# microsoft/VidTok

Hardware: AMD Instinct MI355X
Metric: encode+decode frames/sec, vidtok_kl_causal_488_4chn 17x256x256 (higher is better)
Workload: dtype bf16; 1 GPU; vidtok_kl_causal_488_4chn forward (encode+KL+decode), bf16, B=4 clips/GPU, 17x256x256; global_batch=4, launch=hipGraph replay (engine graph cache)

## Files before the change

### include/vidtok_amd.h

```cpp
#ifndef VIDTOK_AMD_H
#define VIDTOK_AMD_H

#include <stddef.h>
#include <stdint.h>

#ifdef __cplusplus
extern "C" {
#endif

typedef void* vt_stream;

typedef enum vt_status {
  VT_OK = 0,
  VT_ERR_ARG = -1,
  VT_ERR_HIP = -2,
  VT_ERR_UNSUPPORTED = -3
} vt_status;

typedef enum vt_dtype { VT_F32 = 0, VT_BF16 = 1, VT_I32 = 2, VT_BF16X3 = 3 , VT_F16 = 4 } vt_dtype;

typedef enum vt_tmode {
  VT_TPAD_ZERO = 0,
  VT_TPAD_REPLICATE = 1,
  VT_TPAD_CACHE = 2,
// ... 36 lines not shown
  int32_t ldy;
  int32_t KT, KH, KW;
  int32_t st, sh, sw;
  int32_t pt, ph, pw;
  int32_t tmode, ncache;
  int32_t ups_t, ups_s;
  int32_t res_mode;
  int32_t res_tshift;
  int32_t Tr, ldr;
  int32_t out_layout;
  int32_t t_trim;
  int32_t dtype;
  int32_t out_dtype;
  int32_t nbatch;
  int32_t ln_mode;
  int32_t ln_keep_y;
  int32_t ldn;
  int32_t yt_mul, yt_off;
  int32_t ys_mul, ys_oh, ys_ow;
  float ln_eps;
  int64_t xs_z, ws_z, ys_z, rs_z;
  void* work;
  int64_t work_bytes;
} vt_conv_desc;

int vt_conv(const vt_conv_desc* d, vt_stream stream);
int64_t vt_conv_work_bytes(const vt_conv_desc* d);
int vt_conv_plan(const vt_conv_desc* d, int32_t* out8);
int vt_conv_profile(const vt_conv_desc* d, uint64_t* stamps_out, vt_stream stream);
int vt_conv_desc_size(void);

int vt_time_upsample3_supported(const vt_conv_desc* u);
int vt_time_upsample3(const vt_conv_desc* u, const void* v, int32_t ldv, vt_stream stream);

typedef struct vt_tblock_desc {
  const void* x;
  void* y;
  void* n_out;
  const void* w1; const float* b1;
  const void* w2; const float* b2;
  const float* norm1_gamma; const float* norm1_beta;
  const float* norm2_gamma; const float* norm2_beta;
  const float* next_gamma; const float* next_beta;
  int32_t dtype;
  int32_t C, ld;
  int32_t B, T;
  int64_t HW;
  int32_t tmode;
  int32_t keep_y;
  int32_t ln_next_mode;
  float eps;
  int32_t cache_offset;
  void* cache1;
  void* cache2;
} vt_tblock_desc;

int vt_tblock_desc_size(void);
int vt_temporal_block_supported(const vt_tblock_desc* d);
int vt_temporal_block(const vt_tblock_desc* d, vt_stream stream);
int vt_temporal_block_profile(const vt_tblock_desc* d, uint64_t* stamps_out, vt_stream stream);

int vt_layernorm_act(const void* x, int in_dtype, int64_t ldx, void* y, int out_dtype, int64_t ldy,
                     const float* gamma, const float* beta, int64_t M, int32_t C, float eps,
                     int32_t silu, vt_stream stream);

typedef enum { VT_GN_FRAME = 0, VT_GN_PIXEL = 1, VT_GN_CLIP = 2 } vt_gn_scope;
// ... 214 lines not shown
```

### vidtok_amd/csrc/conv_igemm.hip

```cpp
#include <algorithm>
#include <atomic>
#include <type_traits>

#include "conv_select.h"

namespace {

template <typename H>
__global__ __launch_bounds__(256) void splitk_reduce_kernel(const float* __restrict__ part, int planes, long long M, int Cout, const float* __restrict__ bias,
                                                            const H* __restrict__ res, H* __restrict__ y) {
  const long long n8 = M * (Cout / 8);
  const long long plane = M * (long long)Cout;
  for (long long i = (long long)blockIdx.x * blockDim.x + threadIdx.x; i < n8; i += (long long)gridDim.x * blockDim.x) {
    const long long e = i * 8;
    const int c = (int)(e % Cout);
    float v[8];
    {
      const f32x4 a = *reinterpret_cast<const f32x4*>(part + e), b = *reinterpret_cast<const f32x4*>(part + e + 4);
#pragma unroll
      for (int k = 0; k < 4; ++k) { v[k] = a[k]; v[4 + k] = b[k]; }
    }
    for (int pz = 1; pz < planes; ++pz) {
      const f32x4 a = *reinterpret_cast<const f32x4*>(part + pz * plane + e), b = *reinterpret_cast<const f32x4*>(part + pz * plane + e + 4);
#pragma unroll
      for (int k = 0; k < 4; ++k) { v[k] += a[k]; v[4 + k] += b[k]; }
    }
    if (bias) {
      const f32x4 a = *reinterpret_cast<const f32x4*>(bias + c), b = *reinterpret_cast<const f32x4*>(bias + c + 4);
#pragma unroll
      for (int k = 0; k < 4; ++k) { v[k] += a[k]; v[4 + k] += b[k]; }
    }
    if (res) {
      Oct<H> r;
      r.load(res + e);
#pragma unroll
      for (int k = 0; k < 8; ++k) v[k] = r.get(k) + v[k];
    }
    Oct<H>::store(y + e, v);
  }
}

int launch_igemm(int dtype, bool out_f32, const ConvArgs& a, const IgemmVariant& v, int nbatch, void* stream) {
  switch (dtype) {
    case VT_F32: return vt_igemm_dispatch_f32(&a, &v, nbatch, stream);
    case VT_BF16X3: return vt_igemm_dispatch_x3(&a, &v, nbatch, stream);
    case VT_F16: return vt_igemm_dispatch_f16(&a, &v, nbatch, out_f32 ? 1 : 0, stream);
    default: return vt_igemm_dispatch_bf16(&a, &v, nbatch, out_f32 ? 1 : 0, stream);
  }
}

bool splitk_runs(const ConvPlan& p, const ConvArgs& a, const vt_conv_desc* d, bool sized) {
  if (p.kernel != CONV_IGEMM || p.splitk_planes == 0 || d->work == nullptr) return false;
  return !sized || (d->work_bytes >= (int64_t)p.splitk_planes * a.M * a.Cout * 4 && (reinterpret_cast<uintptr_t>(d->work) & 15) == 0);
}

int launch_splitk(const vt_conv_desc* d, const ConvArgs& a_in, const ConvPlan& p, hipStream_t stream) {
  const int planes = p.splitk_planes;
  ConvArgs a = a_in;
  a.ksplit = a.KT == 3 ? 1 : 2;
  a.plane_bytes = (unsigned)((a.KT == 3 ? a.KH * a.KW : a.KW) * a.Cin * 2);
  a.y = reinterpret_cast<char*>(d->work);
  a.bias = nullptr;
  a.res = nullptr; a.res_mode = VT_RES_NONE;
  a.ln_mode = 0;
  a.xs_z = 0; a.ws_z = 0; a.rs_z = 0;
  a.ys_z = (long long)a.M * a.ldy;
  int rc = launch_igemm(d->dtype, true, a, p.split, planes, stream);
  if (rc != VT_OK) return rc;
  const long long n8 = (long long)a.M * (a.Cout / 8);
  const unsigned grid = (unsigned)std::min<long long>((n8 + 255) / 256, 4096);
  const void* res = a_in.res_mode == VT_RES_ADD ? a_in.res : nullptr;
  if (d->dtype == VT_F16)
    hipLaunchKernelGGL(splitk_reduce_kernel<f16_t>, dim3(grid), dim3(256), 0, stream, reinterpret_cast<const float*>(d->work), planes, (long long)a.M, a.Cout, a_in.bias,
                       reinterpret_cast<const f16_t*>(res), reinterpret_cast<f16_t*>(a_in.y));
  else
    hipLaunchKernelGGL(splitk_reduce_kernel<bf16_t>, dim3(grid), dim3(256), 0, stream, reinterpret_cast<const float*>(d->work), planes, (long long)a.M, a.Cout, a_in.bias,
                       reinterpret_cast<const bf16_t*>(res), reinterpret_cast<bf16_t*>(a_in.y));
  VT_CHECK_LAUNCH();
  return VT_OK;
}

}

extern "C" int vt_conv_max_lds_bytes(void) { return 163840; }

extern "C" int vt_conv_plan(const vt_conv_desc* d, int32_t* out8) {
  VT_CHECK_ARG(out8 != nullptr, "vt_conv_plan: null output");
  ConvArgs a;
  ConvPlan p;
  const int rc = conv_decide(d, a, p);
  if (rc != VT_OK) return rc;
  out8[4] = p.ln_fused ? 1 : 0;
  out8[5] = 1;
  out8[6] = p.kernel;
  out8[7] = 0;
  switch (p.kernel) {
    case CONV_NARROW:
      vt_conv_narrow_plan(&a, out8);
      out8[5] = p.narrow_mode == 2 ? 2 : 1;
      break;
    case CONV_WS2:
      out8[0] = 64; out8[1] = 128; out8[2] = 8;
      out8[3] = (a.Wo / 16) * (a.Ho / 4) * a.B * a.To;
      break;
    case CONV_IN8:
      out8[0] = 128; out8[1] = 128; out8[2] = 4;
      out8[3] = a.M / 128;
      out8[7] = 1;
      break;
    case CONV_IGEMM: {
      const TileShape& t = kTileShapes[p.igemm.tile];
      out8[0] = t.bm(); out8[1] = t.bn(); out8[2] = t.waves();
// ... 16 lines not shown
  a.prof_mode = vt_opt(OPT_WS_PROF_MODE);
  if (p.kernel == CONV_WS2) return vt_ws2_launch(&a, d->dtype, stream_);
  VT_CHECK_ARG(p.kernel == CONV_IGEMM && ((d->dtype == VT_BF16 && d->out_dtype == VT_BF16) || d->dtype == VT_BF16X3) && d->ln_mode == 0 &&
                   p.igemm.tile == TILE_256x256,
               "vt_conv_profile: bf16 / split-bf16 launches on the 256 x 256 tile without LayerNorm, or on the weight-stationary kernel");
  return launch_igemm(d->dtype, false, a, p.igemm, p.nbatch, stream_);
}

extern "C" int64_t vt_conv_work_bytes(const vt_conv_desc* d) {
  ConvArgs a;
  ConvPlan p;
  if (conv_decide(d, a, p) != VT_OK || p.kernel != CONV_IGEMM) return 0;
  return (int64_t)p.splitk_planes * a.M * a.Cout * 4;
}

extern "C" int vt_conv(const vt_conv_desc* d, vt_stream stream_) {
  ConvArgs a;
  ConvPlan p;
  int rc = conv_decide(d, a, p);
  if (rc != VT_OK) return rc;
  switch (p.kernel) {
    case CONV_WS2: return vt_ws2_launch(&a, d->dtype, stream_);
    case CONV_NARROW: return vt_conv_narrow_launch(&a, stream_, p.narrow_mode);
    case CONV_IN8: return vt_conv_in8_launch(&a, d->dtype, stream_);
    case CONV_IGEMM: break;
  }
  rc = splitk_runs(p, a, d, true) ? launch_splitk(d, a, p, reinterpret_cast<hipStream_t>(stream_))
                                  : launch_igemm(d->dtype, d->out_dtype == VT_F32, a, p.igemm, p.nbatch, stream_);
  if (rc != VT_OK || d->ln_mode == 0 || p.ln_fused) return rc;
  return vt_layernorm_act(d->y, d->out_dtype, d->ldy, d->ln_out, d->out_dtype, d->ldn, d->ln_gamma, d->ln_beta, a.M, d->Cout,
                          d->ln_eps, d->ln_mode == 2 ? 1 : 0, stream_);
}

extern "C" int vt_time_upsample3_supported(const vt_conv_desc* u) {
  ConvArgs a;
  ConvPlan p;
  if (conv_decide(u, a, p) != VT_OK) return 0;
  return tup3_eligible(u, a, p) ? 1 : 0;
}

extern "C" int vt_time_upsample3(const vt_conv_desc* u, const void* v, int32_t ldv, vt_stream stream_) {
  ConvArgs a;
  ConvPlan p;
  const int rc = conv_decide(u, a, p);
  if (rc != VT_OK) return rc;
  VT_CHECK_ARG(tup3_eligible(u, a, p), "vt_time_upsample3: descriptor not covered (ask vt_time_upsample3_supported; the parity launches of vt_conv serve it)");
  VT_CHECK_ARG(v != nullptr && (reinterpret_cast<uintptr_t>(v) & 15) == 0 && ldv >= u->Cout && ldv % 8 == 0,
               "vt_time_upsample3: v must be 16-byte aligned with ldv = %d >= Cout and a multiple of 8", ldv);
  a.pair_v = reinterpret_cast<const char*>(v);
  a.ldv = ldv;
  const IgemmVariant pair = {TILE_256x256, true, 2, 2, kRowBytes};
  return launch_igemm(u->dtype, false, a, pair, 1, stream_);
}

extern "C" int vt_conv_act(const vt_conv_desc* d, int32_t act, vt_stream stream_) {
  VT_CHECK_ARG(act == VT_ACT_RELU, "vt_conv_act: act %d (VT_ACT_RELU = %d is the one activation)", act, VT_ACT_RELU);
  ConvArgs a;
  ConvPlan p;
  const int rc = conv_decide(d, a, p, nullptr, act);
  if (rc != VT_OK) return rc;
  VT_CHECK_ARG(d->dtype != VT_BF16X3 && d->out_dtype == d->dtype, "vt_conv_act: fp32, bf16 or fp16 arithmetic with results in the same type");
  VT_CHECK_ARG(d->out_layout == VT_NDHWC && d->res_mode == VT_RES_NONE && d->ln_mode == 0 && p.nbatch == 1 && a.yt_mul == 1 && a.ys_mul == 1,
               "vt_conv_act: NDHWC output without residual, LayerNorm, batching or interleave");
  return vt_igemm_dispatch_relu(&a, &p.igemm, d->dtype, stream_);
}
```

### vidtok_amd/csrc/model.cpp

```cpp
#include <hip/hip_runtime.h>
#include <stdint.h>
#include <string.h>

#include <algorithm>
#include <cmath>
#include <map>
#include <memory>
#include <set>
#include <string>
#include <vector>

#include "../../include/vidtok_amd.h"

void vt_set_error(const char* fmt, ...);

namespace {

struct Fail {
  int code;
};
#define M_CHECK(cond, ...)        \
  do {                            \
    if (!(cond)) {                \
      vt_set_error(__VA_ARGS__);  \
// ... 394 lines not shown
  }
  auto standins = [&](vt_conv_desc& q) {
    if (!c.dry) return;
    q.x = q.w = q.y = (void*)16;
    if (q.res_mode != VT_RES_NONE) q.res = (void*)16;
    if (q.res_mode == VT_RES_MIX) q.mix_factor = (const float*)16;
    if (q.tmode == VT_TPAD_CACHE) q.cache = (void*)16;
    if (q.ln_mode != 0) { q.ln_gamma = q.ln_beta = (const float*)16; q.ln_out = (void*)16; }
  };
  if (o.ln_optional && d.ln_mode != 0) {
    vt_conv_desc q = d;
    standins(q);
    int32_t plan[8];
    if (q.ln_out == nullptr) q.ln_out = (void*)16;
    if (!(vt_conv_plan(&q, plan) == VT_OK && plan[4] == 1)) {
      d.ln_gamma = d.ln_beta = nullptr; d.ln_out = nullptr; d.ln_mode = 0;
      r.n = Tens(); r.norm = nullptr;
    }
  }
  if (o.tup3_probe) {
    vt_conv_desc q = d;
    standins(q);
    if (q.ln_mode != 0 && q.ln_out == nullptr) q.ln_out = (void*)16;
    r.tup3 = vt_time_upsample3_supported(&q) == 1;
  }
  if (o.plan_only) return r;
  if (o.tup3_v) {
    if (!c.dry) M_CALL(vt_time_upsample3(&d, o.tup3_v->p, o.tup3_v->ld, c.stream));
    return r;
  }
  {
    vt_conv_desc q = d;
    standins(q);
    const int64_t wb = ((x.dt == VT_BF16 || x.dt == VT_F16) && (g.kt == 3 || g.kh == 3)) ? vt_conv_work_bytes(&q) : 0;
    if (wb > 0) {
      d.work = c.cur->alloc((size_t)wb, c.dry);
      d.work_bytes = wb;
    }
  }
  if (!c.dry) M_CALL(vt_conv(&d, c.stream));
  if (ln_after) {
    M_CHECK(!o.out && !o.ncthw, "vt_model: GroupNorm of an interleaved / NCTHW result");
    r.n = o.ln.norm->of(c, r.y, o.ln.silu, cout);
    r.norm = o.ln.norm; r.silu = o.ln.silu;
  }
  return r;
}

void gather(Ctx& c, const char* src, int Ts, char* dst, int Td, int t0, const std::vector<int>& idx, int B, int64_t frame_elems, int es) {
  for (size_t j0 = 0; j0 < idx.size(); j0 += 128) {
    int32_t part[128];
    const int n = (int)std::min<size_t>(128, idx.size() - j0);
    for (int j = 0; j < n; ++j) part[j] = idx[j0 + j];
    if (!c.dry)
      M_CALL(vt_gather_frames(src, dst + (size_t)(t0 + (int)j0) * frame_elems * es, es, B, frame_elems, (int64_t)Ts * frame_elems, (int64_t)Td * frame_elems, part, n, c.stream));
  }
}

void update_cache(Ctx& c, CState& st, const Tens& x, int P) {
  if (P == 0) return;
  Model* m = c.m;
  const int T = x.T, off = st.offset, es = (int)esize(x.dt);
  const int64_t fr = (int64_t)x.H * x.W * x.ld;
  std::vector<int> sx, sc;
  int jx = -1, jc = -1;
  for (int j = 0; j < P; ++j) {
    const int q = T - off + j;
    M_CHECK(q >= 0, "vt_model: chunk of %d frames is shorter than its cache offset %d", T, off);
    if (q >= P) { if (jx < 0) jx = j; sx.push_back(q - P); }
    else if (m->first_chunk) { if (jx < 0) jx = j; sx.push_back(0); }
// ... 1419 lines not shown
```

### vidtok_amd/csrc/options.cpp

```cpp
#include "options.h"

#include <stdlib.h>
#include <string.h>

#include <atomic>
#include <mutex>

#include "../../include/vidtok_amd.h"

void vt_set_error(const char* fmt, ...);

namespace {
struct OptDef {
  const char* name;
  int dflt;
};
const OptDef kDefs[OPT_COUNT] = {
    {"conv_buf", 1},        {"conv_tinner", 1},     {"conv_ldsepi", 1},      {"conv_ws", 2},
    {"conv_narrow", 1},     {"conv_tile", 0},       {"conv_tile_min", 128},  {"conv_fuse_ln", 1}, {"conv_fuse_ln256", 1},
    {"tblock_fused", 1},    {"tblock_prof_mode", 0},
    {"conv_deep", 1},       {"ws_prof_mode", 0},    {"attn_flash", 1},      {"conv_splitk", 1},
    {"conv_tskip", 1},      {"conv_in8", 1},        {"conv_tup_ln", 1},     {"conv_nt_mb", 64},
    {"conv_tup3", 1},
};
std::atomic<int> g_val[OPT_COUNT];
std::once_flag g_once;

int env_default(int id) {
  char var[64] = "VT_";
  size_t n = 3;
  for (const char* s = kDefs[id].name; *s && n + 1 < sizeof(var); ++s) var[n++] = (*s >= 'a' && *s <= 'z') ? (char)(*s - 32) : *s;
  var[n] = 0;
  const char* e = getenv(var);
  return e ? atoi(e) : kDefs[id].dflt;
}
void init_all() {
  for (int i = 0; i < OPT_COUNT; ++i) g_val[i].store(env_default(i), std::memory_order_relaxed);
}
int find(const char* name) {
  if (!name) return -1;
  for (int i = 0; i < OPT_COUNT; ++i)
    if (strcmp(name, kDefs[i].name) == 0) return i;
  return -1;
}
}

int vt_opt(int id) {
  std::call_once(g_once, init_all);
  return g_val[id].load(std::memory_order_relaxed);
}

extern "C" int vt_set_option(const char* name, int32_t value) {
  const int id = find(name);
  if (id < 0) {
    vt_set_error("vt_set_option: unknown option '%s'", name ? name : "(null)");
    return VT_ERR_ARG;
// ... 25 lines not shown
```

### vidtok_amd/csrc/options.h

```cpp
#pragma once

enum VtOpt {
  OPT_CONV_BUF = 0,
  OPT_CONV_TINNER,
  OPT_CONV_LDSEPI,
  OPT_CONV_WS,
  OPT_CONV_NARROW,
  OPT_CONV_TILE,
  OPT_CONV_TILE_MIN,
  OPT_CONV_FUSE_LN,
  OPT_CONV_FUSE_LN256,
  OPT_TBLOCK_FUSED,
  OPT_TBLOCK_PROF_MODE,
  OPT_CONV_DEEP,
  OPT_WS_PROF_MODE,
  OPT_ATTN_FLASH,
  OPT_CONV_SPLITK,
  OPT_CONV_TSKIP,
  OPT_CONV_IN8,
  OPT_CONV_TUP_LN,
  OPT_CONV_NT_MB,
  OPT_CONV_TUP3,
  OPT_COUNT
};

int vt_opt(int id);
```

### vidtok_amd/lib.py

```python
import ctypes as C
import os

import torch

_HERE = os.path.dirname(os.path.abspath(__file__))
LIB_PATH = os.path.join(_HERE, "libvidtok_amd.so")

VT_F32, VT_BF16, VT_I32, VT_BF16X3, VT_F16 = 0, 1, 2, 3, 4
VT_TPAD_ZERO, VT_TPAD_REPLICATE, VT_TPAD_CACHE, VT_TPAD_ZERO_BACK = 0, 1, 2, 3
VT_GN_FRAME, VT_GN_PIXEL, VT_GN_CLIP = 0, 1, 2
VT_RES_NONE, VT_RES_ADD, VT_RES_MIX = 0, 1, 2
VT_NDHWC, VT_NCTHW = 0, 1
VT_ACT_RELU = 1
VT_LPIPS_CLAMP_Y, VT_LPIPS_ROUNDTRIP, VT_LPIPS_UNIT = 1, 2, 4
VT_SESSION_ENCODE, VT_SESSION_DECODE = 0, 1


class VtError(RuntimeError):
    pass


class ConvDesc(C.Structure):

    _fields_ = (
# ... 91 lines not shown
    "vt_create": (C.c_int, [C.POINTER(ModelConfig), _I32, C.POINTER(_P)]),
    "vt_destroy": (C.c_int, [_P]),
    "vt_load_weight": (C.c_int, [_P, C.c_char_p, _P, C.POINTER(_I64), _I32]),
    "vt_weight_count": (C.c_int, [_P]),
    "vt_weight_name": (C.c_char_p, [_P, _I32]),
    "vt_weight_shape": (C.c_int, [_P, _I32, C.POINTER(_I64), C.POINTER(_I32)]),
    "vt_workspace_bytes": (_I64, [_P, _I32, _I32, _I32, _I32]),
    "vt_latent_dims": (C.c_int, [_P, _I32, _I32, _I32, C.POINTER(_I32)]),
    "vt_encode": (C.c_int, [_P, _P, _I32, _I32, _I32, _I32, _P, _P, _I64, _P]),
    "vt_regularize_kl": (C.c_int, [_P, _P, _P, _P, _P, _I32, _I32, _I32, _I32, _P]),
    "vt_regularize_fsq": (C.c_int, [_P, _P, _P, _P, _I32, _I32, _I32, _I32, _P]),
    "vt_indices_to_latent": (C.c_int, [_P, _P, _P, _I32, _I32, _I32, _I32, _P]),
    "vt_decode": (C.c_int, [_P, _P, _I32, _I32, _I32, _I32, _P, _P, _I64, _P]),
    "vt_reset_cache": (C.c_int, [_P]),
    "vt_prepare": (C.c_int, [_P]),
    "vt_regularize_fsq_aux": (C.c_int, [_P, _P, _I32, _I32, _I32, _I32, _F, _P, _P, _P]),
    "vt_tile_latent_frames": (_I32, [_P, _I32, _I32]),
    "vt_tile_workspace_bytes": (_I64, [_P, _I32, _I32, _I32, _I32, _I32, _I32]),
    "vt_tile_encode": (C.c_int, [_P, _P, _I32, _I32, _I32, _I32, _I32, _P, _P, _I64, _P]),
    "vt_tile_decode": (C.c_int, [_P, _P, _I32, _I32, _I32, _I32, _I32, _I32, _P, _P, _I64, _P]),
    "vt_session_create": (C.c_int, [_P, _I32, _I32, _I32, _I32, _I32, _I32, C.POINTER(_P)]),
    "vt_session_workspace_bytes": (_I64, [_P]),
    "vt_session_push": (C.c_int, [_P, _P, _I32, _P, _I32, C.POINTER(_I32), _P, _I64, _P]),
    "vt_session_finish": (C.c_int, [_P, _P, _I32, C.POINTER(_I32), _P, _I64, _P]),
    "vt_session_destroy": (C.c_int, [_P]),
    "vt_copy_segments": (C.c_int, [_P, _I32, _I64, _P]),
    "vt_conv": (C.c_int, [C.POINTER(ConvDesc), _P]),
    "vt_conv_desc_size": (C.c_int, []),
    "vt_conv_work_bytes": (_I64, [C.POINTER(ConvDesc)]),
    "vt_conv_plan": (C.c_int, [C.POINTER(ConvDesc), C.POINTER(_I32)]),
    "vt_conv_profile": (C.c_int, [C.POINTER(ConvDesc), _P, _P]),
    "vt_time_upsample3_supported": (C.c_int, [C.POINTER(ConvDesc)]),
    "vt_time_upsample3": (C.c_int, [C.POINTER(ConvDesc), _P, _I32, _P]),
    "vt_frames_work_floats": (_I64, [_I32, _I32, _I32]),
    "vt_frames_u8_to_ncthw": (C.c_int, [_P, _I32, _I32, _I32, _I32, _I32, _I32, _I32, _P, _I32, _I32, _I32, _I32, _P, _P]),
    "vt_ncthw_to_frames_u8": (C.c_int, [_P, _I32, _I32, _I32, _I32, _I32, _P, _I32, _I32, _P]),
    "vt_ncthw_copy_frames": (C.c_int, [_P, _P, _I32, _I32, _I32, _I32, _I32, _I32, _I64, _I32, _P]),
    "vt_tblock_desc_size": (C.c_int, []),
    "vt_temporal_block_supported": (C.c_int, [C.POINTER(TBlockDesc)]),
    "vt_temporal_block": (C.c_int, [C.POINTER(TBlockDesc), _P]),
    "vt_temporal_block_profile": (C.c_int, [C.POINTER(TBlockDesc), _P, _P]),
    "vt_flash_attention_supported": (C.c_int, [_I32, _I32, _I32, _I32]),
    "vt_flash_attention": (C.c_int, [_P, _P, _P, _P, _P, _I32, _I32, _I32, _I32, _I32, _F, _P]),
    "vt_layernorm_act": (C.c_int, [_P, C.c_int, _I64, _P, C.c_int, _I64, _P, _P, _I64, _I32, _F, _I32, _P]),
    "vt_tanh_inplace": (C.c_int, [_P, _I64, _P]),
    "vt_softmax_rows": (C.c_int, [_P, _P, C.c_int, _I64, _I32, _I64, _F, _P]),
    "vt_ncthw_to_ndhwc": (C.c_int, [_P, _P, C.c_int, _I32, _I32, _I32, _I32, _I32, _I32, _I32, _P]),
    "vt_ndhwc_to_ncthw": (C.c_int, [_P, C.c_int, _P, _I32, _I32, _I32, _I32, _I32, _I32, _I32, _P]),
    "vt_time_avgpool3s2": (C.c_int, [_P, _P, _P, C.c_int, _I32, _I32, _I64, _I32, _I32, _P]),
    "vt_time_lerp2x": (C.c_int, [_P, _P, C.c_int, _I32, _I32, _I64, _P]),
    "vt_time_lerp2x_cat": (C.c_int, [_P, _I32, _P, _P, C.c_int, _I32, _I32, _I32, _I64, _P]),
    "vt_pack_conv_weight": (C.c_int, [_P, _P, _I32, _I32, _I32, _I32, _I32, _I32, C.POINTER(_I32), _I64, _P]),
    "vt_fsq_consts": (C.c_int, [C.POINTER(_I32), _I32, C.POINTER(_F)]),
    "vt_kl_sample": (C.c_int, [_P, _P, _P, _P, _I32, _I32, _I64, _P]),
    "vt_fsq_quantize": (C.c_int, [_P, _P, _P, C.POINTER(_I32), _I32, _I32, _I64, _P]),
    "vt_fsq_indices_to_codes": (C.c_int, [_P, _P, C.POINTER(_I32), _I32, _I32, _I64, _P]),
    "vt_fsq_quantize_cb": (C.c_int, [_P, _P, _P, C.POINTER(_I32), _I32, _I32, _I32, _I64, _P]),
    "vt_fsq_indices_to_codes_cb": (C.c_int, [_P, _P, C.POINTER(_I32), _I32, _I32, _I32, _I64, _P]),
    "vt_fsq_aux_work_floats": (_I64, [C.POINTER(_I32), _I32, _I32, _I64]),
    "vt_fsq_aux_stats": (C.c_int, [_P, C.POINTER(_I32), _I32, _I32, _I64, _F, _P, _P, _P]),
    "vt_fsq_aux_stats_avg": (C.c_int, [_P, C.POINTER(_I32), _I32, _I32, _I64, _F, _P, _P, _P, _P]),
    "vt_entropy": (C.c_int, [_P, _I64, _P, _P]),
    "vt_fsq_aux_loss": (C.c_int, [_P, _P, _F, _F, _F, _P, _P]),
    "vt_groupnorm_work_bytes": (_I64, [_I32, _I32, _I32, _I32]),
    "vt_groupnorm_act": (C.c_int, [_P, C.c_int, _I64, _P, C.c_int, _I64, _P, _P, _I32, _I32, _I64, _I32, _I32, _I32,
                                   C.c_float, _I32, _P, _P]),
# ... 91 lines not shown
```

### vidtok_amd/ops.py

```python
import ctypes as C
from dataclasses import dataclass
from typing import Optional

import torch

from . import lib as L

_DT = {torch.float32: L.VT_F32, torch.bfloat16: L.VT_BF16, torch.float16: L.VT_F16}
H16 = (torch.bfloat16, torch.float16)
CH_ALIGN = 8


CONV_RECORD = None


def _conv_launch(lib, d, what, keep=()):
    L.check(lib.vt_conv(C.byref(d), _stream()), what)
    if CONV_RECORD is not None:
        CONV_RECORD.append((d, keep, (d.B * d.To * d.Ho * d.Wo * max(1, d.nbatch), d.Cout, d.KT * d.KH * d.KW * d.Cin)))


class TimeUp3Desc(L.ConvDesc):

    v_ptr = None
    ldv = 0


def time_upsample3_supported(d) -> bool:
    return bool(L.load().vt_time_upsample3_supported(C.byref(d)))


def conv_plan(d):
    out = (C.c_int32 * 8)()
    L.check(L.load().vt_conv_plan(C.byref(d), out), "vt_conv_plan")
    return dict(tile=(out[0], out[1]), waves=out[2], workgroups=out[3], ln_fused=bool(out[4]), launches=out[5],
                kernel={2: "narrow", 3: "ws2", 4: "in8"}.get(out[6], "igemm"), lds_epilogue=out[7] == 1, deep_ring=out[7] == 2)


def replay_convs(record, conv_kernel_only=True):
    lib = L.load()
    for d, _keep, _label in record:
        if isinstance(d, L.TBlockDesc):
            L.check(lib.vt_temporal_block(C.byref(d), _stream()), "vt_temporal_block(replay)")
            continue
        if isinstance(d, tuple):
            _, q, k, vT, bias, o, scale = d
            L.check(lib.vt_flash_attention(_ptr(q), _ptr(k), _ptr(vT), _ptr(bias), _ptr(o), _DT[q.dtype], q.shape[0], q.shape[1], q.shape[2],
                                           vT.shape[2], scale, _stream()), "vt_flash_attention(replay)")
            continue
        if isinstance(d, TimeUp3Desc):
            L.check(lib.vt_time_upsample3(C.byref(d), C.c_void_p(d.v_ptr), d.ldv, _stream()), "vt_time_upsample3(replay)")
            continue
        if conv_kernel_only and d.ln_mode != 0 and not conv_plan(d)["ln_fused"]:
            d2 = L.ConvDesc()
            C.memmove(C.byref(d2), C.byref(d), C.sizeof(d))
            d2.ln_mode = 0
            d = d2
        L.check(lib.vt_conv(C.byref(d), _stream()), "vt_conv(replay)")


def pad_channels(c: int) -> int:
    return (c + CH_ALIGN - 1) // CH_ALIGN * CH_ALIGN


def _stream():
    return C.c_void_p(torch.cuda.current_stream().cuda_stream)


def _ptr(t: Optional[torch.Tensor]):
    return None if t is None else C.c_void_p(t.data_ptr())


def _chk(t: torch.Tensor, name: str):
    if not t.is_cuda:
        raise L.VtError(f"{name}: tensor is on {t.device}; vidtok_amd runs on the GPU only (no CPU fallback)")
    if not t.is_contiguous():
        raise L.VtError(f"{name}: tensor must be contiguous")


@dataclass(frozen=True)
class ConvGeom:

    kt: int = 1
    kh: int = 1
    kw: int = 1
    st: int = 1
    sh: int = 1
    sw: int = 1
    pt: int = 0
    ph: int = 0
    pw: int = 0
# ... 72 lines not shown
    if out_s is not None:
        assert out is not None and mul == 1
        d.ys_mul, d.ys_oh, d.ys_ow = 2, int(out_s[0]), int(out_s[1])
    n = None
    if ln is not None:
        gamma, beta, eps, silu = ln
        assert out_layout == L.VT_NDHWC and gamma.dtype == torch.float32 and beta.dtype == torch.float32
        assert gamma.numel() >= cout and beta.numel() >= cout and gamma.is_cuda and beta.is_cuda
        d.ln_gamma, d.ln_beta, d.ln_out = gamma.data_ptr(), beta.data_ptr(), y.data_ptr()
        d.ln_mode, d.ln_keep_y, d.ldn, d.ln_eps = (2 if silu else 1), int(bool(ln_keep_y)), ldy, float(eps)
        fused = True
        if ln_optional:
            try:
                fused = conv_plan(d)["ln_fused"]
            except L.VtError:
                fused = False
        if fused:
            if callable(ln_out):
                ln_out = ln_out()
            if ln_out is not None:
                assert ln_out.shape == y.shape and ln_out.dtype == out_dtype and ln_out.is_contiguous()
                n = ln_out
            else:
                n = (torch.zeros if ldy != cout else torch.empty)(y.shape, dtype=out_dtype, device=x.device)
            d.ln_out = n.data_ptr()
        else:
            assert ln_keep_y
            d.ln_gamma = d.ln_beta = d.ln_out = None
            d.ln_mode = 0
            ln, n = None, None
    work = None
    if x.dtype in H16 and (geom.kt == 3 or geom.kh == 3):
        nb = lib.vt_conv_work_bytes(C.byref(d))
        if nb > 0:
            work = torch.empty((nb,), dtype=torch.uint8, device=x.device)
            d.work, d.work_bytes = work.data_ptr(), nb
    _conv_launch(lib, d, "vt_conv", (x, w, bias, y, res, cache, mix_factor, n, ln, work))
    if ln is None:
        return y
    return (y, n) if ln_keep_y else n


TUP3_GEOM = ConvGeom(kt=2, kh=3, kw=3, pt=1, ph=1, pw=1, ph_hi=1, pw_hi=1)


def time_upsample3(x, wu, v, mix_factor, out, *, cout: int, ln=None, ln_out=None):
    if not x.is_cuda or x.dtype not in _DT:
        return None
    lib = L.load()
    _chk(x, "time_upsample3.x"); _chk(out, "time_upsample3.out")
    B, T, H, W, Cin = x.shape
    ld = out.shape[4]
    assert out.dtype == x.dtype and tuple(out.shape[:4]) == (B, 2 * T, H, W) and ld >= cout, (out.shape, x.shape)
    assert mix_factor.dtype == torch.float32 and mix_factor.is_cuda
    g = TUP3_GEOM
    d = TimeUp3Desc()
    d.x, d.w, d.y = x.data_ptr(), x.data_ptr(), out.data_ptr()
    d.B, d.Ti, d.Hi, d.Wi, d.Cin = B, T, H, W, Cin
    d.To, d.Ho, d.Wo, d.Cout = T, H, W, cout
    d.ldw, d.ldy = g.kt * g.kh * g.kw * Cin, ld
    d.KT, d.KH, d.KW, d.st, d.sh, d.sw, d.pt, d.ph, d.pw = g.kt, g.kh, g.kw, 1, 1, 1, g.pt, g.ph, g.pw
    d.tmode = L.VT_TPAD_ZERO
    d.res_mode, d.res, d.res_tshift, d.Tr, d.ldr, d.mix_factor = L.VT_RES_MIX, x.data_ptr(), 0, T, Cin, mix_factor.data_ptr()
    d.out_layout, d.dtype, d.out_dtype, d.nbatch = L.VT_NDHWC, _DT[x.dtype], _DT[x.dtype], 1
    d.yt_mul, d.yt_off = 2, 0
    if ln is not None:
        gamma, beta, eps, silu = ln
# ... 139 lines not shown
        x.shape, dtype=out_dtype, device=x.device)
    assert gamma.dtype == torch.float32 and beta.dtype == torch.float32 and gamma.numel() == c
    L.check(lib.vt_layernorm_act(_ptr(x), _DT[x.dtype], ld, _ptr(y), _DT[out_dtype], ld, _ptr(gamma), _ptr(beta),
                                 M, c, float(eps), int(bool(silu)), _stream()), "vt_layernorm_act")
    if LN_RECORD is not None:
        LN_RECORD.append((x, y, gamma, beta, M, c, float(eps), bool(silu)))
    return y


def replay_layernorms(record):
    lib = L.load()
    for x, y, gamma, beta, M, c, eps, silu in record:
        ld = x.shape[-1]
        L.check(lib.vt_layernorm_act(_ptr(x), _DT[x.dtype], ld, _ptr(y), _DT[y.dtype], ld, _ptr(gamma), _ptr(beta), M, c, eps,
                                     int(silu), _stream()), "vt_layernorm_act(replay)")


def launch_bytes(d):
    if isinstance(d, tuple):
        _, q, k, vT, _b, o, _s = d
        return (q.numel() + k.numel() + vT.numel() + o.numel()) * q.element_size()
    if isinstance(d, L.TBlockDesc):
        es = 2
        px = d.B * d.T * d.HW
        return px * d.ld * es * (1 + (1 if d.keep_y else 0) + (1 if d.ln_next_mode else 0)) + 2 * d.C * 3 * d.C * es
    if isinstance(d, TimeUp3Desc):
        px = d.B * d.To * d.Ho * d.Wo
        return px * d.Cin * 2 + d.Cout * d.ldw * 2 + px * d.Cout * 2 * (1 + 2 + (2 if d.ln_mode != 0 else 0))
    es = 2 if d.dtype in (L.VT_BF16, L.VT_F16) else 4
    eo = 4 if d.out_dtype == L.VT_F32 else 2
    nb = max(1, d.nbatch)
    M = d.B * d.To * d.Ho * d.Wo * nb
    plan = conv_plan(d)
    nbytes = d.B * d.Ti * d.Hi * d.Wi * d.Cin * es * (nb if d.xs_z or nb == 1 else 1) + d.Cout * d.ldw * es * nb
    if not (d.ln_mode != 0 and plan["ln_fused"] and not d.ln_keep_y):
        nbytes += M * d.Cout * eo
    if d.res_mode != L.VT_RES_NONE:
        nbytes += M * d.Cout * eo
    if d.ln_mode != 0 and plan["ln_fused"]:
        nbytes += M * d.Cout * eo
    return nbytes


def launch_class(d):
    if isinstance(d, tuple):
        return None
    if isinstance(d, L.TBlockDesc):
        return "temporal block fused (C=128)", launch_bytes(d)
    taps = d.KT * d.KH * d.KW
    if conv_plan(d)["kernel"] == "narrow":
        name = "conv_out 3x3x3 128->3 (conv3d_narrow_kernel)"
    elif taps == 1 and d.nbatch <= 1:
        name = "1x1 convolutions (nin_shortcut, attention projections)"
    elif d.Cin <= 8:
        name = "conv_in 3x3x3 (3 -> C)"
    elif d.KH == 1 and d.KW == 1 and d.KT == 3 and d.Cin <= 256:
        name = f"temporal k3 convolutions, unfused (C={d.Cin})"
    else:
        return None
    return name, launch_bytes(d)


GN_POS = 3


def groupnorm_act(x, gamma, beta, *, scope, silu, eps=1e-6, out_dtype=None, c=None, groups=32):
# ... 636 lines not shown
```

Before: 967.1 frames/s.

## Fuse LayerNorm into split-K reduce for 3-tap convs with LN epilogue

```diff
diff --git a/include/vidtok_amd.h b/include/vidtok_amd.h
--- a/include/vidtok_amd.h
+++ b/include/vidtok_amd.h
@@ -92,6 +92,9 @@
 
 int vt_time_upsample3_supported(const vt_conv_desc* u);
 int vt_time_upsample3(const vt_conv_desc* u, const void* v, int32_t ldv, vt_stream stream);
+
+int vt_conv_splitk_ln_supported(const vt_conv_desc* d);
+int vt_conv_splitk_ln(const vt_conv_desc* d, vt_stream stream);
 
 typedef struct vt_tblock_desc {
   const void* x;
diff --git a/vidtok_amd/csrc/conv_igemm.hip b/vidtok_amd/csrc/conv_igemm.hip
--- a/vidtok_amd/csrc/conv_igemm.hip
+++ b/vidtok_amd/csrc/conv_igemm.hip
@@ -40,6 +40,57 @@
   }
 }
 
+template <typename H, int G, bool SILU>
+__global__ __launch_bounds__(256) void splitk_reduce_ln_kernel(const float* __restrict__ part, int planes, long long M, const float* __restrict__ bias,
+                                                               const H* __restrict__ res, H* __restrict__ y, const float* __restrict__ gamma,
+                                                               const float* __restrict__ beta, H* __restrict__ n, int ldn, float eps) {
+  constexpr int Cout = 8 * G;
+  const long long n8 = M * G;
+  const long long plane = M * (long long)Cout;
+  const int c = (int)(threadIdx.x % G) * 8;
+  float lg[8], lb[8], bq[8];
+#pragma unroll
+  for (int h = 0; h < 2; ++h) {
+    const f32x4 g4 = *reinterpret_cast<const f32x4*>(gamma + c + 4 * h), b4 = *reinterpret_cast<const f32x4*>(beta + c + 4 * h);
+    f32x4 q4 = {0.0f, 0.0f, 0.0f, 0.0f};
+    if (bias) q4 = *reinterpret_cast<const f32x4*>(bias + c + 4 * h);
+#pragma unroll
+    for (int k = 0; k < 4; ++k) {
+      lg[4 * h + k] = ln_fold(g4[k], SILU);
+      lb[4 * h + k] = ln_fold(b4[k], SILU);
+      bq[4 * h + k] = q4[k];
+    }
+  }
+  for (long long i = (long long)blockIdx.x * blockDim.x + threadIdx.x; i < n8; i += (long long)gridDim.x * blockDim.x) {
+    const long long e = i * 8;
+    float v[8];
+    {
+      const f32x4 a = *reinterpret_cast<const f32x4*>(part + e), b = *reinterpret_cast<const f32x4*>(part + e + 4);
+#pragma unroll
+      for (int k = 0; k < 4; ++k) { v[k] = a[k]; v[4 + k] = b[k]; }
+    }
+    for (int pz = 1; pz < planes; ++pz) {
+      const f32x4 a = *reinterpret_cast<const f32x4*>(part + pz * plane + e), b = *reinterpret_cast<const f32x4*>(part + pz * plane + e + 4);
+#pragma unroll
+      for (int k = 0; k < 4; ++k) { v[k] += a[k]; v[4 + k] += b[k]; }
+    }
+    if (bias) {
+#pragma unroll
+      for (int k = 0; k < 8; ++k) v[k] += bq[k];
+    }
+    if (res) {
+      Oct<H> r;
+      r.load(res + e);
+#pragma unroll
+      for (int k = 0; k < 8; ++k) v[k] = r.get(k) + v[k];
+    }
+    if (y) Oct<H>::store(y + e, v);
+    float o[8];
+    ln_row8<G, SILU>(v, lg, lb, eps, o);
+    Oct<H>::store(n + (i / G) * ldn + c, o);
+  }
+}
+
 int launch_igemm(int dtype, bool out_f32, const ConvArgs& a, const IgemmVariant& v, int nbatch, void* stream) {
   switch (dtype) {
     case VT_F32: return vt_igemm_dispatch_f32(&a, &v, nbatch, stream);
@@ -54,8 +105,7 @@
   return !sized || (d->work_bytes >= (int64_t)p.splitk_planes * a.M * a.Cout * 4 && (reinterpret_cast<uintptr_t>(d->work) & 15) == 0);
 }
 
-int launch_splitk(const vt_conv_desc* d, const ConvArgs& a_in, const ConvPlan& p, hipStream_t stream) {
-  const int planes = p.splitk_planes;
+int launch_splitk_planes(const vt_conv_desc* d, const ConvArgs& a_in, const ConvPlan& p, hipStream_t stream) {
   ConvArgs a = a_in;
   a.ksplit = a.KT == 3 ? 1 : 2;
   a.plane_bytes = (unsigned)((a.KT == 3 ? a.KH * a.KW : a.KW) * a.Cin * 2);
@@ -65,19 +115,62 @@
   a.ln_mode = 0;
   a.xs_z = 0; a.ws_z = 0; a.rs_z = 0;
   a.ys_z = (long long)a.M * a.ldy;
-  int rc = launch_igemm(d->dtype, true, a, p.split, planes, stream);
+  return launch_igemm(d->dtype, true, a, p.split, p.splitk_planes, stream);
+}
+
+int launch_splitk(const vt_conv_desc* d, const ConvArgs& a, const ConvPlan& p, hipStream_t stream) {
+  const int planes = p.splitk_planes;
+  int rc = launch_splitk_planes(d, a, p, stream);
   if (rc != VT_OK) return rc;
   const long long n8 = (long long)a.M * (a.Cout / 8);
   const unsigned grid = (unsigned)std::min<long long>((n8 + 255) / 256, 4096);
-  const void* res = a_in.res_mode == VT_RES_ADD ? a_in.res : nullptr;
+  const void* res = a.res_mode == VT_RES_ADD ? a.res : nullptr;
   if (d->dtype == VT_F16)
-    hipLaunchKernelGGL(splitk_reduce_kernel<f16_t>, dim3(grid), dim3(256), 0, stream, reinterpret_cast<const float*>(d->work), planes, (long long)a.M, a.Cout, a_in.bias,
-                       reinterpret_cast<const f16_t*>(res), reinterpret_cast<f16_t*>(a_in.y));
+    hipLaunchKernelGGL(splitk_reduce_kernel<f16_t>, dim3(grid), dim3(256), 0, stream, reinterpret_cast<const float*>(d->work), planes, (long long)a.M, a.Cout, a.bias,
+                       reinterpret_cast<const f16_t*>(res), reinterpret_cast<f16_t*>(a.y));
   else
-    hipLaunchKernelGGL(splitk_reduce_kernel<bf16_t>, dim3(grid), dim3(256), 0, stream, reinterpret_cast<const float*>(d->work), planes, (long long)a.M, a.Cout, a_in.bias,
-                       reinterpret_cast<const bf16_t*>(res), reinterpret_cast<bf16_t*>(a_in.y));
+    hipLaunchKernelGGL(splitk_reduce_kernel<bf16_t>, dim3(grid), dim3(256), 0, stream, reinterpret_cast<const float*>(d->work), planes, (long long)a.M, a.Cout, a.bias,
+                       reinterpret_cast<const bf16_t*>(res), reinterpret_cast<bf16_t*>(a.y));
   VT_CHECK_LAUNCH();
   return VT_OK;
+}
+
+bool splitk_ln_eligible(const vt_conv_desc* d, const ConvArgs& a, const ConvPlan& p) {
+  if (vt_opt(OPT_CONV_SPLITK_LN) == 0 || (d->ln_mode != 1 && d->ln_mode != 2)) return false;
+  if (!vt_is_h16(d->dtype) || d->out_dtype != d->dtype) return false;
+  if (d->Cout != 128 && d->Cout != 256 && d->Cout != 512) return false;
+  if (d->ldy != d->Cout || d->ldn < d->Cout || d->ldn % 8 != 0) return false;
+  if (!d->ln_gamma || !d->ln_beta || !d->ln_out || (reinterpret_cast<uintptr_t>(d->ln_out) & 15) || (reinterpret_cast<uintptr_t>(d->y) & 15)) return false;
+  if (a.res_mode == VT_RES_ADD && (reinterpret_cast<uintptr_t>(a.res) & 15)) return false;
+  if ((reinterpret_cast<uintptr_t>(d->ln_gamma) & 15) || (reinterpret_cast<uintptr_t>(d->ln_beta) & 15) || (reinterpret_cast<uintptr_t>(d->bias) & 15)) return false;
+  return splitk_runs(p, a, d, true);
+}
+
+int decide_without_ln(const vt_conv_desc* d, ConvArgs& a, ConvPlan& p) {
+  VT_CHECK_ARG(d != nullptr, "vt_conv: null descriptor");
+  vt_conv_desc q = *d;
+  q.ln_mode = 0;
+  return conv_decide(&q, a, p);
+}
+
+template <typename H, int G>
+void launch_reduce_ln(const vt_conv_desc* d, const ConvArgs& a, int planes, hipStream_t stream) {
+  const long long n8 = (long long)a.M * G;
+  const unsigned grid = (unsigned)std::min<long long>((n8 + 1023) / 1024, 4096);
+  const H* res = a.res_mode == VT_RES_ADD ? reinterpret_cast<const H*>(a.res) : nullptr;
+  H* y = d->ln_keep_y ? reinterpret_cast<H*>(a.y) : nullptr;
+  if (d->ln_mode == 2)
+    hipLaunchKernelGGL((splitk_reduce_ln_kernel<H, G, true>), dim3(grid), dim3(256), 0, stream, reinterpret_cast<const float*>(d->work), planes, (long long)a.M,
+                       a.bias, res, y, d->ln_gamma, d->ln_beta, reinterpret_cast<H*>(d->ln_out), d->ldn, d->ln_eps);
+  else
+    hipLaunchKernelGGL((splitk_reduce_ln_kernel<H, G, false>), dim3(grid), dim3(256), 0, stream, reinterpret_cast<const float*>(d->work), planes, (long long)a.M,
+                       a.bias, res, y, d->ln_gamma, d->ln_beta, reinterpret_cast<H*>(d->ln_out), d->ldn, d->ln_eps);
+}
+template <typename H>
+void launch_reduce_ln(const vt_conv_desc* d, const ConvArgs& a, int planes, hipStream_t stream) {
+  if (a.Cout == 128) launch_reduce_ln<H, 16>(d, a, planes, stream);
+  else if (a.Cout == 256) launch_reduce_ln<H, 32>(d, a, planes, stream);
+  else launch_reduce_ln<H, 64>(d, a, planes, stream);
 }
 
 }
@@ -160,6 +253,28 @@
                           d->ln_eps, d->ln_mode == 2 ? 1 : 0, stream_);
 }
 
+extern "C" int vt_conv_splitk_ln_supported(const vt_conv_desc* d) {
+  ConvArgs a;
+  ConvPlan p;
+  if (d == nullptr || d->ln_mode == 0 || decide_without_ln(d, a, p) != VT_OK) return 0;
+  return splitk_ln_eligible(d, a, p) ? 1 : 0;
+}
+
+extern "C" int vt_conv_splitk_ln(const vt_conv_desc* d, vt_stream stream_) {
+  ConvArgs a;
+  ConvPlan p;
+  int rc = decide_without_ln(d, a, p);
+  if (rc != VT_OK) return rc;
+  VT_CHECK_ARG(splitk_ln_eligible(d, a, p), "vt_conv_splitk_ln: descriptor not covered (ask vt_conv_splitk_ln_supported; vt_conv serves it)");
+  hipStream_t stream = reinterpret_cast<hipStream_t>(stream_);
+  rc = launch_splitk_planes(d, a, p, stream);
+  if (rc != VT_OK) return rc;
+  if (d->dtype == VT_F16) launch_reduce_ln<f16_t>(d, a, p.splitk_planes, stream);
+  else launch_reduce_ln<bf16_t>(d, a, p.splitk_planes, stream);
+  VT_CHECK_LAUNCH();
+  return VT_OK;
+}
+
 extern "C" int vt_time_upsample3_supported(const vt_conv_desc* u) {
   ConvArgs a;
   ConvPlan p;
diff --git a/vidtok_amd/csrc/model.cpp b/vidtok_amd/csrc/model.cpp
--- a/vidtok_amd/csrc/model.cpp
+++ b/vidtok_amd/csrc/model.cpp
@@ -450,10 +450,29 @@
   {
     vt_conv_desc q = d;
     standins(q);
-    const int64_t wb = ((x.dt == VT_BF16 || x.dt == VT_F16) && (g.kt == 3 || g.kh == 3)) ? vt_conv_work_bytes(&q) : 0;
-    if (wb > 0) {
-      d.work = c.cur->alloc((size_t)wb, c.dry);
-      d.work_bytes = wb;
+    const bool taps3 = (x.dt == VT_BF16 || x.dt == VT_F16) && (g.kt == 3 || g.kh == 3);
+    const int64_t wb = taps3 ? vt_conv_work_bytes(&q) : 0;
+    int64_t wl = 0;
+    int32_t opt_ln = 0;
+    if (taps3 && d.ln_mode != 0 && vt_get_option("conv_splitk_ln", &opt_ln) == VT_OK && opt_ln != 0) {
+      q.ln_mode = 0;
+      wl = vt_conv_work_bytes(&q);
+      q.ln_mode = d.ln_mode;
+    }
+    bool split_ln = false;
+    if (wb > 0 || wl > 0) {
+      d.work = c.cur->alloc((size_t)std::max(wb, wl), c.dry);
+      d.work_bytes = std::max(wb, wl);
+      if (wl > 0) {
+        q.work = c.dry ? (void*)256 : d.work;
+        q.work_bytes = d.work_bytes;
+        split_ln = vt_conv_splitk_ln_supported(&q) == 1;
+      }
+      if (!split_ln && wb == 0) { d.work = nullptr; d.work_bytes = 0; }
+    }
+    if (split_ln) {
+      if (!c.dry) M_CALL(vt_conv_splitk_ln(&d, c.stream));
+      return r;
     }
   }
   if (!c.dry) M_CALL(vt_conv(&d, c.stream));
diff --git a/vidtok_amd/csrc/options.cpp b/vidtok_amd/csrc/options.cpp
--- a/vidtok_amd/csrc/options.cpp
+++ b/vidtok_amd/csrc/options.cpp
@@ -21,7 +21,7 @@
     {"tblock_fused", 1},    {"tblock_prof_mode", 0},
     {"conv_deep", 1},       {"ws_prof_mode", 0},    {"attn_flash", 1},      {"conv_splitk", 1},
     {"conv_tskip", 1},      {"conv_in8", 1},        {"conv_tup_ln", 1},     {"conv_nt_mb", 64},
-    {"conv_tup3", 1},
+    {"conv_tup3", 1},       {"conv_splitk_ln", 1},
 };
 std::atomic<int> g_val[OPT_COUNT];
 std::once_flag g_once;
diff --git a/vidtok_amd/csrc/options.h b/vidtok_amd/csrc/options.h
--- a/vidtok_amd/csrc/options.h
+++ b/vidtok_amd/csrc/options.h
@@ -21,6 +21,7 @@
   OPT_CONV_TUP_LN,
   OPT_CONV_NT_MB,
   OPT_CONV_TUP3,
+  OPT_CONV_SPLITK_LN,
   OPT_COUNT
 };
 
diff --git a/vidtok_amd/lib.py b/vidtok_amd/lib.py
--- a/vidtok_amd/lib.py
+++ b/vidtok_amd/lib.py
@@ -147,6 +147,8 @@
     "vt_conv_profile": (C.c_int, [C.POINTER(ConvDesc), _P, _P]),
     "vt_time_upsample3_supported": (C.c_int, [C.POINTER(ConvDesc)]),
     "vt_time_upsample3": (C.c_int, [C.POINTER(ConvDesc), _P, _I32, _P]),
+    "vt_conv_splitk_ln_supported": (C.c_int, [C.POINTER(ConvDesc)]),
+    "vt_conv_splitk_ln": (C.c_int, [C.POINTER(ConvDesc), _P]),
     "vt_frames_work_floats": (_I64, [_I32, _I32, _I32]),
     "vt_frames_u8_to_ncthw": (C.c_int, [_P, _I32, _I32, _I32, _I32, _I32, _I32, _I32, _P, _I32, _I32, _I32, _I32, _P, _P]),
     "vt_ncthw_to_frames_u8": (C.c_int, [_P, _I32, _I32, _I32, _I32, _I32, _P, _I32, _I32, _P]),
diff --git a/vidtok_amd/ops.py b/vidtok_amd/ops.py
--- a/vidtok_amd/ops.py
+++ b/vidtok_amd/ops.py
@@ -14,8 +14,19 @@
 CONV_RECORD = None
 
 
+def splitk_ln_supported(d) -> bool:
+    return d.ln_mode != 0 and bool(L.load().vt_conv_splitk_ln_supported(C.byref(d)))
+
+
+def _run_conv(lib, d, what):
+    if splitk_ln_supported(d):
+        L.check(lib.vt_conv_splitk_ln(C.byref(d), _stream()), what.replace("vt_conv", "vt_conv_splitk_ln"))
+    else:
+        L.check(lib.vt_conv(C.byref(d), _stream()), what)
+
+
 def _conv_launch(lib, d, what, keep=()):
-    L.check(lib.vt_conv(C.byref(d), _stream()), what)
+    _run_conv(lib, d, what)
     if CONV_RECORD is not None:
         CONV_RECORD.append((d, keep, (d.B * d.To * d.Ho * d.Wo * max(1, d.nbatch), d.Cout, d.KT * d.KH * d.KW * d.Cin)))
 
@@ -56,7 +67,7 @@
             C.memmove(C.byref(d2), C.byref(d), C.sizeof(d))
             d2.ln_mode = 0
             d = d2
-        L.check(lib.vt_conv(C.byref(d), _stream()), "vt_conv(replay)")
+        _run_conv(lib, d, "vt_conv(replay)")
 
 
 def pad_channels(c: int) -> int:
@@ -195,7 +206,16 @@
     work = None
     if x.dtype in H16 and (geom.kt == 3 or geom.kh == 3):
         nb = lib.vt_conv_work_bytes(C.byref(d))
-        if nb > 0:
+        if d.ln_mode != 0 and L.get_option("conv_splitk_ln") != 0:
+            mode, d.ln_mode = d.ln_mode, 0
+            nb_ln = lib.vt_conv_work_bytes(C.byref(d))
+            d.ln_mode = mode
+            if nb_ln > 0:
+                work = torch.empty((nb_ln,), dtype=torch.uint8, device=x.device)
+                d.work, d.work_bytes = work.data_ptr(), nb_ln
+                if not splitk_ln_supported(d):
+                    work, d.work, d.work_bytes = None, None, 0
+        if work is None and nb > 0:
             work = torch.empty((nb,), dtype=torch.uint8, device=x.device)
             d.work, d.work_bytes = work.data_ptr(), nb
     _conv_launch(lib, d, "vt_conv", (x, w, bias, y, res, cache, mix_factor, n, ln, work))
@@ -401,6 +421,8 @@
     nb = max(1, d.nbatch)
     M = d.B * d.To * d.Ho * d.Wo * nb
     plan = conv_plan(d)
+    if splitk_ln_supported(d):
+        plan = dict(plan, ln_fused=True)
     nbytes = d.B * d.Ti * d.Hi * d.Wi * d.Cin * es * (nb if d.xs_z or nb == 1 else 1) + d.Cout * d.ldw * es * nb
     if not (d.ln_mode != 0 and plan["ln_fused"] and not d.ln_keep_y):
         nbytes += M * d.Cout * eo
```

Measured after the change: 967.8 frames/s (median of 3 runs). No clear change (+0.1%).
